# topling/toplingdb

Hardware: NVIDIA H100
Metric: compaction_input_kv_MB_per_s (higher is better)
Workload: dtype u8

## Files before the change

toplingdb_b200/csrc/api.cu:

```cuda
#include <cuda_runtime.h>
#include <stdio.h>
#include <stdlib.h>
#include <string.h>

#include <algorithm>
#include <map>
#include <memory>
#include <mutex>
#include <unordered_map>
#include <string>
#include <thread>
#include <type_traits>
#include <vector>

#include "../../include/b200c.h"
#include "inflate_rules.h"
#include "kernels.h"
#include "range_plan.h"
#include "scan.cuh"
#include "sst_host.h"

using namespace b200c;

namespace {
// ... 190 lines not shown
  cudaEvent_t a, b;
  float us;
};

}

struct b200c_job {
  b200c_params p;
  std::vector<uint64_t> snapshots, fct;
  std::string cf_name, db_id, db_session_id, db_host_id;
  std::vector<Input> inputs;
  std::vector<Output> outputs;
  b200c_stats stats;
  int stage_done = 0;
  uint64_t launches = 0;
  int sms = 132;
  cudaStream_t st = nullptr;
  cudaStream_t st2 = nullptr;
  cudaStream_t st_up = nullptr;
  cudaEvent_t ev[5] = {nullptr, nullptr, nullptr, nullptr, nullptr};
  cudaEvent_t evx[4] = {nullptr, nullptr, nullptr, nullptr};
  DevBuf files_d, blk_off, blk_size, blk_state, scan_tmp, run_start, small;
  KeyBufs dec, mrg;
  DevBuf splits, tile_state, snaps_d;
  DevBuf esz, eshared, tstat, nxt, disk, rows, tstate, grows, gstate, gflag, gsync, idx_contrib, idx_contrib_off, blocks, files_rec, idx_esz, idx_eoff, idx_sep, out_buf, out_base_d;
  uint64_t n_total = 0, n_out = 0, nblk_in = 0, nblocks_out = 0;
  uint32_t nfiles_out = 0, nruns = 0;
  DevBuf bloom_contrib, bloom_contrib_off;
  DevBuf bloom_hashes;
  DevBuf kv_arena, kv_offs, kv_klens;
  DevBuf run_bounds, run_first_d;
  std::vector<uint64_t> run_start_h;
  HostBuf host_out;
  std::vector<GpKey> gp_small, gp_large;
  std::vector<uint64_t> gp_size;
  std::vector<uint8_t> gp_same;
  DevBuf gp_keys_d, gp_ranks_d, gp_size_d, gp_same_d, gp_cuts_d;
  BoundKey range_lo{}, range_hi{};
  DevBuf clip_d;
  DevBuf cslot, cslot_off, arena;
  std::vector<cudaEvent_t> range_events;
  std::vector<std::string> range_bounds;
  cudaEvent_t wait_ev = nullptr;
  DevBuf vfiles_d, vrun_start;
  HostBuf pin_small, pin_tails, pin_rd, pin_up;
  size_t pin_up_used = 0;
  std::vector<KernelTime> ktimes;
// ... 721 lines not shown
  uint32_t maxb = 0;
  for (auto& f : fds) maxb = std::max(maxb, f.nblocks);
  if (nblk) {
    j->kt_begin("decode.index");
    launch_index_decode(files_d, k, maxb, j->blk_off.as<uint64_t>(), j->blk_size.as<uint32_t>(), j->range_lo, P.has_range_start, j->range_hi,
                        P.has_range_end, err, st);
    j->kt_end();
    j->launches++;
  }
  const uint8_t* arena = nullptr;
  if (nblk && any_compressed) {
    CU(j->cslot.reserve(4 * (nblk + 1)));
    CU(j->cslot_off.reserve(8 * (nblk + 1)));
    j->kt_begin("decode.inflate");
    launch_block_usize(files_d, j->blk_off.as<uint64_t>(), j->blk_size.as<uint32_t>(), (uint32_t)nblk, j->cslot.as<uint32_t>(), err, st);
    exclusive_scan<uint32_t>(j->cslot.as<uint32_t>(), j->cslot_off.as<uint64_t>(), nblk, j->scan_tmp.as<uint64_t>(), small + kSlotArena, st, &j->launches);
    uint64_t hc[kSmallSlots];
    if (int rc = checked_sync(j, hc)) return rc;
    CU(j->arena.reserve(hc[kSlotArena] + 256));
    arena = j->arena.as<uint8_t>();
    launch_inflate_blocks(files_d, j->blk_off.as<uint64_t>(), j->blk_size.as<uint32_t>(), j->cslot.as<uint32_t>(), j->cslot_off.as<uint64_t>(),
                          (uint32_t)nblk, j->arena.as<uint8_t>(), P.verify_input_checksums, err, j->sms, st);
    j->kt_end();
    j->launches += 3;
  }
  CU(cudaMemsetAsync(j->run_start.p, 0, 8 * (k + 1), st));
  if (nblk) {
    CU(cudaMemsetAsync(j->blk_state.p, 0, 8 * (nblk + 1), st));
    j->kt_begin("decode.blocks");
    launch_block_decode_fused(files_d, k, j->blk_off.as<uint64_t>(), j->blk_size.as<uint32_t>(), (uint32_t)nblk, P.verify_input_checksums, N,
                              j->dec.mut(), j->blk_state.as<unsigned long long>(), reinterpret_cast<uint32_t*>(small + kSlotDecTicket),
                              j->run_start.as<uint64_t>(), small + kSlotTotalIn, err, j->sms, st, arena);
    j->kt_end();
    j->launches++;
  }
  CU(cudaEventRecord(j->ev[1], st));
  const KeyCols decc = j->dec.cols(N);
  if (until == 1) {
    uint64_t h[kSmallSlots];
    j->run_start_h.resize(k + 1);
    CU(cudaMemcpyAsync(j->run_start_h.data(), j->run_start.p, 8 * (k + 1), cudaMemcpyDeviceToHost, st));
    if (int rc = checked_sync(j, h)) return rc;
    if (h[kSlotTotalIn] != N && !(P.has_range_start || P.has_range_end))
      return fail(B200C_ERR_CORRUPTION, "decoded entry count differs from rocksdb.num.entries");
    j->stage_done = 1;
    j->stats.kernel_launches = j->launches;
    return B200C_OK;
// ... 20 lines not shown
    j->kt_begin("merge.clip");
    launch_clip_runs(decc, runs, K, j->range_lo, P.has_range_start, j->range_hi, P.has_range_end,
                     j->clip_d.as<uint64_t>(), reinterpret_cast<unsigned long long*>(small + kSlotClip), st);
    j->kt_end();
    j->launches++;
    uint64_t hc[kSmallSlots];
    if (int rc = checked_sync(j, hc)) return rc;
    N_in = hc[kSlotClip];
    range_value_bytes = hc[kSlotClip + 1];
    if (N_in > n_decoded) return fail(B200C_ERR_CUDA, "internal: clipped entry count exceeds the input");
    runs = RunBounds{j->clip_d.as<uint64_t>(), j->clip_d.as<uint64_t>() + K};
    j->stats.num_input_records = N_in;
  }
  return run_merge_encode(j, until, decc, runs, n_decoded, N_in, clipped, range_value_bytes, small, err);
}

int run_merge_encode(b200c_job* j, int until, KeyCols decc, RunBounds runs, uint64_t n_decoded, uint64_t N, bool clipped,
                     uint64_t range_value_bytes, uint64_t* small, uint32_t* err) {
  const b200c_params& P = j->p;
  cudaStream_t st = j->st;
  const size_t k = j->nruns;
  const uint64_t mtiles = (N + kMergeNominal - 1) / kMergeNominal;
  CU(j->splits.reserve(8 * (mtiles + 1) * k));
  CU(j->tile_state.reserve(8 * (mtiles + 1)));
  CU(cudaMemsetAsync(j->tile_state.p, 0, 8 * (mtiles + 1), st));
  CU(j->snaps_d.reserve(8 * (P.num_snapshots + 1)));
  if (P.num_snapshots)
    if (int rc = upload_small(j, j->snaps_d.p, j->snapshots.data(), 8 * P.num_snapshots)) return rc;
  CU(j->mrg.reserve(N));
  CU(j->esz.reserve(4 * (N + 1)));
  CU(j->eshared.reserve(N + 1));
  CU(j->tstat.reserve(sizeof(TileStat) * (mtiles + 2)));
  MergeParams mp;
  mp.nruns = (uint32_t)k;
  mp.bottommost = P.bottommost_level != 0;
  mp.nsnapshots = P.num_snapshots;
  mp.snapshots = j->snaps_d.as<uint64_t>();
  mp.earliest_snapshot = P.num_snapshots ? j->snapshots[0] : kMaxSeq;
  mp.filter = P.compaction_filter;
  mp.ttl = P.ttl;
  mp.now = P.ttl_now;
  mp.write_conflict_snapshot = P.earliest_write_conflict_snapshot != 0 && P.earliest_write_conflict_snapshot < kMaxSeq;
  MergeCounters* counters = reinterpret_cast<MergeCounters*>(small + kSlotCounters);
  EncodeWork W;
  memset(&W, 0, sizeof W);
  W.esz = j->esz.as<uint32_t>();
  W.eshared = j->eshared.as<uint8_t>();
  W.tstat = j->tstat.as<TileStat>();
  W.min_s1 = reinterpret_cast<uint32_t*>(small + kSlotMinS1);
  W.totals = small + kSlotTotals;
  if (N) {
    j->kt_begin("merge.partition");
    launch_merge_partition(decc, runs, (uint32_t)k, N, mtiles, j->splits.as<uint64_t>(), err, j->sms, st);
    j->kt_end();
    const MergeSizes msz{W.esz, W.eshared, W.tstat, W.min_s1};
    W.tprefix = j->tile_state.as<unsigned long long>();
    W.nstat = mtiles;
    j->kt_begin("merge.tiles");
    launch_merge_tiles(decc, runs, mp, N, mtiles, j->splits.as<uint64_t>(),
                       j->tile_state.as<unsigned long long>(), reinterpret_cast<uint32_t*>(small + kSlotTicket), j->mrg.mut(), counters, msz, err, st);
    j->kt_end();
    j->kt_begin("merge.sizes_fix");
    launch_merge_sizes_fix(j->mrg.cols(0), j->tile_state.as<unsigned long long>(), mtiles, msz, st);
    j->kt_end();
    j->launches += 3;
  }
  CU(cudaEventRecord(j->ev[2], st));
  uint64_t h[kSmallSlots];
  if (int rc = checked_sync(j, h)) return rc;
  if (clipped ? h[kSlotTotalIn] > n_decoded : h[kSlotTotalIn] != n_decoded)
    return fail(B200C_ERR_CORRUPTION, "decoded entry count differs from rocksdb.num.entries");
  MergeCounters mc;
  memcpy(&mc, h + kSlotCounters, sizeof mc);
  const uint64_t n_out = mc.n_out;
  j->n_out = n_out;
  j->stats.num_output_records = n_out;
  j->stats.num_input_deletion_records = mc.n_input_deletions;
  j->stats.num_records_replaced = mc.n_hidden;
  j->stats.num_expired_deletion_records = mc.n_obsolete;
  j->stats.num_record_drop_user = mc.n_user_drop;
  j->stats.total_input_raw_key_bytes = mc.raw_key_bytes;
  {
    uint64_t all = 0;
    for (auto& in : j->inputs) all += in.tail.raw_value_size;
    if (clipped) all = range_value_bytes;
    j->stats.total_input_raw_value_bytes = all - mc.raw_value_bytes;
  }
  if (until == 2) {
// ... 547 lines not shown
```

toplingdb_b200/csrc/kernels.h:

```cpp
#pragma once
#include <cuda_runtime.h>
#include <stdint.h>

#include <atomic>

#include "common.cuh"
#include "gp_rules.h"

namespace b200c {

struct PerDeviceFlag {
  std::atomic<uint64_t> mask{0};
  uint64_t bit_of_current_device() const {
    int d = 0;
    cudaGetDevice(&d);
    return 1ull << (d & 63);
  }
  bool is_set(uint64_t bit) const { return (mask.load(std::memory_order_acquire) & bit) != 0; }
  void set(uint64_t bit) { mask.fetch_or(bit, std::memory_order_release); }
};

struct FileDesc {
  const uint8_t* base;
  uint64_t len;
// ... 54 lines not shown
  int64_t now;
  uint32_t write_conflict_snapshot;
};
struct TileStat {
  uint64_t raw_key, raw_value, deletions, smallest_seq, largest_seq;
};
struct MergeSizes {
  uint32_t* esz;
  uint8_t* eshared;
  TileStat* tstat;
  uint32_t* min_s1;
};
struct MergeCounters {
  unsigned long long n_out, n_input_deletions, n_hidden, n_obsolete, raw_key_bytes, raw_value_bytes, n_silent, n_user_drop;
};
struct RunBounds {
  const uint64_t* begin;
  const uint64_t* end;
};
void launch_clip_runs(KeyCols in, RunBounds runs, uint32_t nruns, BoundKey start, uint32_t has_start, BoundKey end,
                      uint32_t has_end, uint64_t* clip, unsigned long long* totals, cudaStream_t st);
void launch_run_bounds(KeyCols in, const uint64_t* file_start, const uint32_t* run_first, uint32_t nruns, uint64_t* bounds, uint32_t* err,
                       cudaStream_t st);
void launch_merge_partition(KeyCols in, RunBounds runs, uint32_t nruns, uint64_t n_total, uint64_t ntiles,
                            uint64_t* splits, uint32_t* err, int sms, cudaStream_t st);
void launch_merge_tiles(KeyCols in, RunBounds runs, MergeParams mp, uint64_t n_total, uint64_t ntiles,
                        const uint64_t* splits, unsigned long long* tile_state, uint32_t* ticket, KeyColsMut out,
                        MergeCounters* counters, MergeSizes ms, uint32_t* err, cudaStream_t st);
void launch_merge_sizes_fix(KeyCols merged, const unsigned long long* tile_state, uint64_t ntiles, MergeSizes ms, cudaStream_t st);

struct GpCut {
  uint64_t entry;
  uint64_t block_bytes;
};
struct EncodeParams {
  uint32_t block_size, block_size_limit , restart_interval;
  uint32_t checksum, format_version, output_level;
  uint64_t max_output_file_size;
  GpCtx gp;
  GpCut* gp_cuts;
  uint32_t* gp_ncuts;
};
using GpKey = BoundKey;
void launch_bloom_count(KeyCols m, uint64_t n, FileRec* files, const uint64_t* nfiles_dev, uint32_t millibits, uint64_t* hashes, int sms, cudaStream_t st);
void launch_bloom_build(const uint64_t* hashes, uint64_t n, const FileRec* files, uint32_t nfiles, uint32_t max_filter_bytes, uint32_t millibits, uint32_t cksum,
                        uint8_t* const* out_base, uint64_t* contrib, const uint64_t* contrib_off, cudaStream_t st);
void launch_gp_ranks(KeyCols m, const GpKey* smallest, const GpKey* largest, uint32_t n, uint64_t* lo, uint64_t* eq, uint64_t* hi,
                     cudaStream_t st);
// ... 84 lines not shown
```

toplingdb_b200/csrc/merge.cu:

```cuda
#include "common.cuh"
#include "group_rules.h"
#include "kernels.h"

namespace b200c {

constexpr int kMT = kMergeTile;
constexpr int kMThreads = 256;
constexpr int kMV = kMT / kMThreads;

__device__ __forceinline__ Key load_key(const KeyCols& c, uint64_t i) {
  Key k;
  ulonglong2 p = c.pfx[i];
  k.hi = p.x;
  k.lo = p.y;
  k.tr = c.tr[i];
  k.ulen = meta_ulen(c.meta[i]);
  return k;
}

__device__ __forceinline__ uint64_t count_before(const KeyCols& c, uint64_t base, uint64_t lo, uint64_t hi, const Key& x,
                                                 bool before_equal) {
  while (lo < hi) {
    uint64_t mid = lo + ((hi - lo) >> 1);
    Key e = load_key(c, base + mid);
    bool precedes = before_equal ? !ikey_less(x, e) : ikey_less(e, x);
    if (precedes) lo = mid + 1;
    else hi = mid;
  }
  return lo;
}

__global__ void __launch_bounds__(128)
merge_partition_kernel(KeyCols in, RunBounds runs, uint32_t nruns, uint64_t n_total, uint64_t ntiles,
                       uint64_t* __restrict__ splits, uint32_t* __restrict__ err) {
  const unsigned lane = threadIdx.x & 31;
  const uint64_t b = (uint64_t)blockIdx.x * (blockDim.x >> 5) + (threadIdx.x >> 5);
  if (b > ntiles) return;
  uint64_t d = b * (uint64_t)kMergeNominal;
  if (d > n_total) d = n_total;
  uint64_t base[2], lo[2], hi[2];
#pragma unroll
  for (int s = 0; s < 2; s++) {
    uint32_t r = lane + 32 * s;
    base[s] = r < nruns ? runs.begin[r] : 0;
    uint64_t n = r < nruns ? runs.end[r] - runs.begin[r] : 0;
    lo[s] = (d == n_total) ? n : 0;
    hi[s] = (d == 0) ? 0 : n;
  }
  for (int guard = 0; guard < 64 * 70; guard++) {
    unsigned long long best = 0;
#pragma unroll
    for (int s = 0; s < 2; s++) {
      unsigned long long wdt = hi[s] - lo[s];
      unsigned long long enc = (wdt << 7) | (unsigned long long)(lane + 32 * s);
      if (wdt && enc > best) best = enc;
    }
#pragma unroll
    for (int dd = 16; dd; dd >>= 1) {
      unsigned long long o = __shfl_xor_sync(0xffffffffu, best, dd);
      if (o > best) best = o;
    }
    if (best == 0) break;
    const uint32_t p = (uint32_t)(best & 127);
    const int ps = p >> 5, pl = p & 31;
    uint64_t m = ps ? (lo[1] + ((hi[1] - lo[1]) >> 1)) : (lo[0] + ((hi[0] - lo[0]) >> 1));
    m = __shfl_sync(0xffffffffu, m, pl);
    uint64_t pbase = __shfl_sync(0xffffffffu, ps ? base[1] : base[0], pl);
    const Key x = load_key(in, pbase + m);
    uint64_t c[2], sum = 0;
#pragma unroll
    for (int s = 0; s < 2; s++) {
      uint32_t r = lane + 32 * s;
      if (r == p) c[s] = m;
      else if (r < nruns) c[s] = count_before(in, base[s], lo[s], hi[s], x, r < p);
      else c[s] = 0;
      sum += c[s];
    }
#pragma unroll
    for (int dd = 16; dd; dd >>= 1) sum += __shfl_xor_sync(0xffffffffu, sum, dd);
    const bool x_before = sum < d;
#pragma unroll
    for (int s = 0; s < 2; s++) {
      uint32_t r = lane + 32 * s;
      if (r >= nruns) continue;
      if (x_before) lo[s] = (r == p) ? m + 1 : c[s];
      else hi[s] = (r == p) ? m : c[s];
    }
  }
  uint64_t tot = lo[0] + lo[1];
#pragma unroll
  for (int dd = 16; dd; dd >>= 1) tot += __shfl_xor_sync(0xffffffffu, tot, dd);
  if (tot != d && lane == 0) atomicOr(err, kErrKeyOrder);
  if (lane == 0 && (*reinterpret_cast<volatile uint32_t*>(err) & (uint32_t)kFlagHasSingleDelete)) atomicOr(err, (uint32_t)kErrGroupTooLong);
#pragma unroll
  for (int s = 0; s < 2; s++) {
    uint32_t r = lane + 32 * s;
    if (r < nruns) splits[b * nruns + r] = lo[s];
  }
}

constexpr uint32_t kPartStride = 64;
struct GroupLanes {
  uint32_t gshift, g, r, sub, gbase, nruns;
};
__device__ __forceinline__ bool entry_precedes(const KeyCols& c, uint64_t i, const Key& x, bool before_equal) {
  const ulonglong2 p = c.pfx[i];
  if (p.x != x.hi) return p.x < x.hi;
  if (p.y != x.lo) return p.y < x.lo;
  const uint32_t ul = meta_ulen(c.meta[i]);
  if (ul != x.ulen) return ul < x.ulen;
  const uint64_t tr = c.tr[i];
  if (tr != x.tr) return tr > x.tr;
  return before_equal;
}
__device__ __forceinline__ void msel_grouped(const KeyCols& in, const GroupLanes& L, uint64_t base, uint64_t stride, uint64_t d, uint64_t& lo,
                                             uint64_t& hi) {
  const uint32_t g = L.g, r = L.r, sub = L.sub, gbase = L.gbase, gshift = L.gshift;
  for (int guard = 0; guard < 64 * 70; guard++) {
    const unsigned long long wdt = hi - lo;
    unsigned long long best = wdt ? ((wdt << 7) | (unsigned long long)r) : 0;
#pragma unroll
    for (int dd = 16; dd; dd >>= 1) {
      const unsigned long long o = __shfl_xor_sync(0xffffffffu, best, dd);
      if (o > best) best = o;
    }
    if (best == 0) break;
    const uint32_t p = (uint32_t)(best & 127);
    const uint64_t m = __shfl_sync(0xffffffffu, lo + ((hi - lo) >> 1), (int)(p << gshift));
    const uint64_t pbase = __shfl_sync(0xffffffffu, base, (int)(p << gshift));
    const Key x = load_key(in, pbase + m * stride);
    const bool before_equal = r < p;
    uint64_t clo = lo, chi = hi;
    if (r == p) clo = chi = m;
    while (__any_sync(0xffffffffu, chi > clo)) {
      const uint64_t w = chi - clo;
      uint64_t pos = clo;
      bool valid = false;
      if (w > 0) {
        if (w <= g) {
          pos = clo + sub;
          valid = sub < w;
        } else {
          pos = clo + (w * (sub + 1)) / (g + 1);
          valid = true;
        }
      }
      bool prec = false;
      if (valid) prec = entry_precedes(in, base + pos * stride, x, before_equal);
      const unsigned bal = __ballot_sync(0xffffffffu, prec);
      const uint32_t cp = __popc((bal >> gbase) & ((1u << g) - 1u));
      const uint32_t nvalid = w == 0 ? 0 : (w <= g ? (uint32_t)w : g);
      const uint64_t below = __shfl_sync(0xffffffffu, pos, (int)(gbase + (cp ? cp - 1 : 0)));
      const uint64_t above = __shfl_sync(0xffffffffu, pos, (int)(gbase + (cp < g ? cp : g - 1)));
      if (w > 0) {
        if (cp) clo = below + 1;
        if (cp < nvalid) chi = above;
        else if (w <= g) chi = clo;
      }
    }
    const uint64_t c = clo;
    uint64_t sum = sub == 0 ? c : 0;
#pragma unroll
    for (int dd = 16; dd; dd >>= 1) sum += __shfl_xor_sync(0xffffffffu, sum, dd);
    const bool x_before = sum < d;
    if (r < L.nruns) {
      if (x_before) lo = (r == p) ? m + 1 : c;
      else hi = (r == p) ? m : c;
    }
  }
}
__global__ void __launch_bounds__(128, 12)
merge_partition_grouped_kernel(KeyCols in, RunBounds runs, uint32_t nruns, uint32_t gshift, uint64_t n_total,
                               uint64_t ntiles, uint64_t* __restrict__ splits, uint32_t* __restrict__ err, uint32_t chunk) {
  const unsigned lane = threadIdx.x & 31;
  const uint64_t b0 = ((uint64_t)blockIdx.x * (blockDim.x >> 5) + (threadIdx.x >> 5)) * chunk;
  if (b0 > ntiles) return;
  GroupLanes L;
  L.gshift = gshift;
  L.g = 1u << gshift;
  L.r = lane >> gshift;
  L.sub = lane & (L.g - 1);
  L.gbase = L.r << gshift;
  L.nruns = nruns;
  const uint32_t r = L.r, sub = L.sub;
  const uint64_t base = r < nruns ? runs.begin[r] : 0;
  const uint64_t nrun = r < nruns ? runs.end[r] - runs.begin[r] : 0;
  uint64_t prev_lo = 0, prev_d = 0;
  const bool sd_mode = (*reinterpret_cast<volatile uint32_t*>(err) & (uint32_t)kFlagHasSingleDelete) != 0;
  for (uint32_t c = 0; c < chunk; c++) {
    const uint64_t b = b0 + c;
    if (b > ntiles) break;
    uint64_t d = b * (uint64_t)kMergeNominal;
    if (d > n_total) d = n_total;
    uint64_t lo = (d == n_total) ? nrun : 0, hi = (d == 0) ? 0 : nrun;
    if (d != 0 && d != n_total) {
      if (c != 0) {
        lo = prev_lo;
        hi = d > prev_d ? (prev_lo + (d - prev_d) < nrun ? prev_lo + (d - prev_d) : nrun) : prev_lo;
      } else {
        const uint64_t S = kPartStride, msamp = (nrun + S - 1) / S;
        uint64_t M = sub == 0 ? msamp : 0;
#pragma unroll
        for (int dd = 16; dd; dd >>= 1) M += __shfl_xor_sync(0xffffffffu, M, dd);
        const uint64_t T_lo = d / S, T_hi = (d + (S - 1) * (uint64_t)nruns + S - 1) / S;
        uint64_t tlo = 0, tlo_hi = msamp;
        if (T_lo > 0) msel_grouped(in, L, base, S, T_lo, tlo, tlo_hi);
        if (tlo) lo = S * tlo - (S - 1);
        if (T_hi < M) {
          uint64_t thi = tlo, thi_hi = tlo + (T_hi - T_lo) < msamp ? tlo + (T_hi - T_lo) : msamp;
          msel_grouped(in, L, base, S, T_hi, thi, thi_hi);
          const uint64_t h = S * thi;
          hi = h < nrun ? h : nrun;
        }
        if (hi < lo) hi = lo;
      }
    }
    msel_grouped(in, L, base, 1, d, lo, hi);
    uint64_t tot = sub == 0 ? lo : 0;
#pragma unroll
    for (int dd = 16; dd; dd >>= 1) tot += __shfl_xor_sync(0xffffffffu, tot, dd);
    if (tot != d && lane == 0) atomicOr(err, kErrKeyOrder);
    if (sd_mode && d != 0 && d != n_total) {
      Key head, tail;
      head.hi = head.lo = ~0ull, head.ulen = 0xffffffffu, head.tr = 0;
      tail.hi = tail.lo = 0, tail.ulen = 0, tail.tr = ~0ull;
      const bool have_head = r < nruns && sub == 0 && lo < nrun, have_tail = r < nruns && sub == 0 && lo > 0;
      if (have_head) head = load_key(in, base + lo);
      if (have_tail) tail = load_key(in, base + lo - 1);
      Key mh = head, mt = tail;
      bool anyh = have_head, anyt = have_tail;
#pragma unroll
      for (int dd = 16; dd; dd >>= 1) {
        Key oh, ot;
        oh.hi = __shfl_xor_sync(0xffffffffu, mh.hi, dd), oh.lo = __shfl_xor_sync(0xffffffffu, mh.lo, dd), oh.ulen = __shfl_xor_sync(0xffffffffu, mh.ulen, dd);
        ot.hi = __shfl_xor_sync(0xffffffffu, mt.hi, dd), ot.lo = __shfl_xor_sync(0xffffffffu, mt.lo, dd), ot.ulen = __shfl_xor_sync(0xffffffffu, mt.ulen, dd);
        const bool ohv = __shfl_xor_sync(0xffffffffu, (int)anyh, dd) != 0, otv = __shfl_xor_sync(0xffffffffu, (int)anyt, dd) != 0;
        if (ohv && (!anyh || ukey_cmp(oh.hi, oh.lo, oh.ulen, mh.hi, mh.lo, mh.ulen) < 0)) mh = oh, anyh = true;
        if (otv && (!anyt || ukey_cmp(ot.hi, ot.lo, ot.ulen, mt.hi, mt.lo, mt.ulen) > 0)) mt = ot, anyt = true;
      }
      if (anyh && anyt && ukey_cmp(mh.hi, mh.lo, mh.ulen, mt.hi, mt.lo, mt.ulen) == 0) {
        uint32_t adv = 0;
        if (r < nruns && sub == 0) {
          while (lo < nrun && adv <= (uint32_t)kSdSpill) {
            const ulonglong2 p = in.pfx[base + lo];
            if (!same_ukey(mh, p.x, p.y, meta_ulen(in.meta[base + lo]))) break;
            lo++;
            adv++;
          }
        }
        uint32_t tadv = adv;
#pragma unroll
        for (int dd = 16; dd; dd >>= 1) tadv += __shfl_xor_sync(0xffffffffu, tadv, dd);
        if (tadv > (uint32_t)kSdSpill && lane == 0) atomicOr(err, (uint32_t)kErrGroupTooLong);
        d += tadv;
        lo = __shfl_sync(0xffffffffu, lo, (int)L.gbase);
      }
    }
    if (r < nruns && sub == 0) splits[b * nruns + r] = lo;
    prev_lo = lo;
    prev_d = d;
  }
}

constexpr uint32_t kSnapCache = 16;
struct TileSmem {
  uint64_t hi[kMT], lo[kMT], tr[kMT];
  uint16_t idx[kMT];
  uint8_t ulen[kMT];
  uint8_t verd[kMT];
  uint32_t seg[kMaxRuns + 1];
  uint32_t lst[2][kMaxRuns + 2];
  uint64_t sbeg[kMaxRuns];
  uint64_t snaps[kSnapCache];
  unsigned long long red[8];
  unsigned long long stat[5];
  uint32_t smin, smax;
  uint32_t wsum[40];
  uint64_t base_out;
  uint32_t tile_id, kept_total;
  Key pred;
  uint32_t has_pred;
};

__device__ __forceinline__ Key skey(const TileSmem& s, uint32_t id) {
  Key k;
// ... 707 lines not shown
  if ((threadIdx.x & 31) == 0 && sum) atomicAdd(&totals[1], sum);
}
void launch_clip_runs(KeyCols in, RunBounds runs, uint32_t nruns, BoundKey start, uint32_t has_start, BoundKey end,
                      uint32_t has_end, uint64_t* clip, unsigned long long* totals, cudaStream_t st) {
  if (nruns) clip_runs_kernel<<<dim3(kClipSlices, nruns), 256, 0, st>>>(in, runs, nruns, start, has_start, end, has_end, clip, totals);
}
__global__ void run_bounds_kernel(KeyCols in, const uint64_t* __restrict__ file_start, const uint32_t* __restrict__ run_first, uint32_t nruns,
                                  uint64_t* __restrict__ bounds, uint32_t* __restrict__ err) {
  const uint32_t r = blockIdx.x * blockDim.x + threadIdx.x;
  if (r >= nruns) return;
  const uint32_t f0 = run_first[r], f1 = run_first[r + 1];
  bounds[r] = file_start[f0];
  bounds[nruns + r] = file_start[f1];
  for (uint32_t f = f0 + 1; f < f1; f++) {
    const uint64_t e = file_start[f];
    if (e > file_start[f0] && e < file_start[f1] && !ikey_less(load_key(in, e - 1), load_key(in, e))) atomicOr(err, (uint32_t)kErrKeyOrder);
  }
}
void launch_run_bounds(KeyCols in, const uint64_t* file_start, const uint32_t* run_first, uint32_t nruns, uint64_t* bounds, uint32_t* err,
                       cudaStream_t st) {
  if (nruns) run_bounds_kernel<<<(nruns + 63) / 64, 64, 0, st>>>(in, file_start, run_first, nruns, bounds, err);
}

void launch_merge_partition(KeyCols in, RunBounds runs, uint32_t nruns, uint64_t n_total, uint64_t ntiles,
                            uint64_t* splits, uint32_t* err, int sms, cudaStream_t st) {
  unsigned warps = (unsigned)(ntiles + 1);
  if (nruns <= 16) {
    uint32_t kp2 = 2;
    while (kp2 < nruns) kp2 <<= 1;
    uint32_t gshift = 0;
    while ((kp2 << (gshift + 1)) <= 32) gshift++;
    const unsigned wave = (unsigned)sms * 48u;
    uint32_t chunk = (uint32_t)((warps + wave - 1) / wave);
    if (chunk > 4) chunk = 4;
    if (chunk < 1) chunk = 1;
    const unsigned chunks = (warps + chunk - 1) / chunk;
    merge_partition_grouped_kernel<<<(chunks + 3) / 4, 128, 0, st>>>(in, runs, nruns, gshift, n_total, ntiles, splits, err, chunk);
    return;
  }
  merge_partition_kernel<<<(warps + 3) / 4, 128, 0, st>>>(in, runs, nruns, n_total, ntiles, splits, err);
}
static_assert(sizeof(Key) * kMaxRuns <= sizeof(uint64_t) * kMT && 4 * kMaxRuns <= 2 * kMT, "candidate staging must fit");
static_assert(kMergeCtasPerSm * (sizeof(TileSmem) + 1024) <= 227 * 1024, "merge tile must fit three CTAs per SM");
void launch_merge_tiles(KeyCols in, RunBounds runs, MergeParams mp, uint64_t n_total, uint64_t ntiles,
                        const uint64_t* splits, unsigned long long* tile_state, uint32_t* ticket, KeyColsMut out,
                        MergeCounters* counters, MergeSizes ms, uint32_t* err, cudaStream_t st) {
  if (ntiles == 0) return;
  static PerDeviceFlag attr;
  const uint64_t dev_bit = attr.bit_of_current_device();
  if (!attr.is_set(dev_bit)) {
    cudaFuncSetAttribute(merge_tiles_kernel<false>, cudaFuncAttributeMaxDynamicSharedMemorySize, (int)sizeof(TileSmem));
    cudaFuncSetAttribute(merge_tiles_kernel<true>, cudaFuncAttributeMaxDynamicSharedMemorySize, (int)sizeof(TileSmem));
    attr.set(dev_bit);
  }
  merge_tiles_kernel<false><<<(unsigned)ntiles, kMThreads, sizeof(TileSmem), st>>>(in, runs, mp, n_total, ntiles, splits, tile_state, ticket,
                                                                                   out, counters, ms, err);
  merge_tiles_kernel<true><<<(unsigned)ntiles, kMThreads, sizeof(TileSmem), st>>>(in, runs, mp, n_total, ntiles, splits, tile_state, ticket,
                                                                                  out, counters, ms, err);
}
void launch_merge_sizes_fix(KeyCols merged, const unsigned long long* tile_state, uint64_t ntiles, MergeSizes ms, cudaStream_t st) {
  if (ntiles) merge_sizes_fix_kernel<<<(unsigned)((ntiles + 127) / 128), 128, 0, st>>>(merged, tile_state, ntiles, ms);
}

// ... 2 lines not shown
```

Baseline: 281,800.

## Pre-sort sampled fence keys to bound merge partition searches

Replaces the per-tile multi-way selection over sampled keys with a global fence array. Every 64th key of each run is gathered and merged pairwise across runs over log2(nruns) rounds. Each partition warp then indexes the sorted fences directly to get tight per-run bounds before the exact selection. This removes repeated sample-level selection work per tile, at the cost of extra scratch memory and several extra kernel launches.

```diff
diff --git a/toplingdb_b200/csrc/api.cu b/toplingdb_b200/csrc/api.cu
--- a/toplingdb_b200/csrc/api.cu
+++ b/toplingdb_b200/csrc/api.cu
@@ -236,7 +236,7 @@
   cudaEvent_t evx[4] = {nullptr, nullptr, nullptr, nullptr};
   DevBuf files_d, blk_off, blk_size, blk_state, scan_tmp, run_start, small;
   KeyBufs dec, mrg;
-  DevBuf splits, tile_state, snaps_d;
+  DevBuf splits, fences, tile_state, snaps_d;
   DevBuf esz, eshared, tstat, nxt, disk, rows, tstate, grows, gstate, gflag, gsync, idx_contrib, idx_contrib_off, blocks, files_rec, idx_esz, idx_eoff, idx_sep, out_buf, out_base_d;
   uint64_t n_total = 0, n_out = 0, nblk_in = 0, nblocks_out = 0;
   uint32_t nfiles_out = 0, nruns = 0;
@@ -1004,7 +1004,7 @@
     launch_inflate_blocks(files_d, j->blk_off.as<uint64_t>(), j->blk_size.as<uint32_t>(), j->cslot.as<uint32_t>(), j->cslot_off.as<uint64_t>(),
                           (uint32_t)nblk, j->arena.as<uint8_t>(), P.verify_input_checksums, err, j->sms, st);
     j->kt_end();
-    j->launches += 3;
+    j->launches += 2;
   }
   CU(cudaMemsetAsync(j->run_start.p, 0, 8 * (k + 1), st));
   if (nblk) {
@@ -1071,6 +1071,7 @@
   const size_t k = j->nruns;
   const uint64_t mtiles = (N + kMergeNominal - 1) / kMergeNominal;
   CU(j->splits.reserve(8 * (mtiles + 1) * k));
+  CU(j->fences.reserve(merge_partition_scratch_bytes((uint32_t)k, N)));
   CU(j->tile_state.reserve(8 * (mtiles + 1)));
   CU(cudaMemsetAsync(j->tile_state.p, 0, 8 * (mtiles + 1), st));
   CU(j->snaps_d.reserve(8 * (P.num_snapshots + 1)));
@@ -1100,7 +1101,7 @@
   W.totals = small + kSlotTotals;
   if (N) {
     j->kt_begin("merge.partition");
-    launch_merge_partition(decc, runs, (uint32_t)k, N, mtiles, j->splits.as<uint64_t>(), err, j->sms, st);
+    j->launches += launch_merge_partition(decc, runs, (uint32_t)k, N, mtiles, j->fences.p, j->splits.as<uint64_t>(), err, st);
     j->kt_end();
     const MergeSizes msz{W.esz, W.eshared, W.tstat, W.min_s1};
     W.tprefix = j->tile_state.as<unsigned long long>();
@@ -1112,7 +1113,7 @@
     j->kt_begin("merge.sizes_fix");
     launch_merge_sizes_fix(j->mrg.cols(0), j->tile_state.as<unsigned long long>(), mtiles, msz, st);
     j->kt_end();
-    j->launches += 3;
+    j->launches += 2;
   }
   CU(cudaEventRecord(j->ev[2], st));
   uint64_t h[kSmallSlots];
diff --git a/toplingdb_b200/csrc/kernels.h b/toplingdb_b200/csrc/kernels.h
--- a/toplingdb_b200/csrc/kernels.h
+++ b/toplingdb_b200/csrc/kernels.h
@@ -100,8 +100,9 @@
                       uint32_t has_end, uint64_t* clip, unsigned long long* totals, cudaStream_t st);
 void launch_run_bounds(KeyCols in, const uint64_t* file_start, const uint32_t* run_first, uint32_t nruns, uint64_t* bounds, uint32_t* err,
                        cudaStream_t st);
-void launch_merge_partition(KeyCols in, RunBounds runs, uint32_t nruns, uint64_t n_total, uint64_t ntiles,
-                            uint64_t* splits, uint32_t* err, int sms, cudaStream_t st);
+size_t merge_partition_scratch_bytes(uint32_t nruns, uint64_t n_total);
+int launch_merge_partition(KeyCols in, RunBounds runs, uint32_t nruns, uint64_t n_total, uint64_t ntiles, void* scratch,
+                           uint64_t* splits, uint32_t* err, cudaStream_t st);
 void launch_merge_tiles(KeyCols in, RunBounds runs, MergeParams mp, uint64_t n_total, uint64_t ntiles,
                         const uint64_t* splits, unsigned long long* tile_state, uint32_t* ticket, KeyColsMut out,
                         MergeCounters* counters, MergeSizes ms, uint32_t* err, cudaStream_t st);
diff --git a/toplingdb_b200/csrc/merge.cu b/toplingdb_b200/csrc/merge.cu
--- a/toplingdb_b200/csrc/merge.cu
+++ b/toplingdb_b200/csrc/merge.cu
@@ -30,151 +30,242 @@
   return lo;
 }
 
-__global__ void __launch_bounds__(128)
-merge_partition_kernel(KeyCols in, RunBounds runs, uint32_t nruns, uint64_t n_total, uint64_t ntiles,
-                       uint64_t* __restrict__ splits, uint32_t* __restrict__ err) {
+constexpr uint32_t kPartStride = 64;
+constexpr int kFenceWin = 1024;
+constexpr int kFenceThreads = 256;
+
+struct FenceCols {
+  ulonglong2* pfx;
+  uint64_t* tr;
+  uint32_t* ulen;
+  uint32_t* ord[2];
+  uint64_t* foff;
+};
+__device__ __forceinline__ Key fence_key(const FenceCols& fc, uint64_t f) {
+  Key k;
+  const ulonglong2 p = fc.pfx[f];
+  k.hi = p.x;
+  k.lo = p.y;
+  k.tr = fc.tr[f];
+  k.ulen = fc.ulen[f];
+  return k;
+}
+__device__ __forceinline__ uint32_t fence_at(const uint32_t* ord, uint64_t i) { return ord ? ord[i] : (uint32_t)i; }
+
+__global__ void __launch_bounds__(kFenceThreads)
+merge_fence_gather_kernel(KeyCols in, RunBounds runs, uint32_t nruns, FenceCols fc) {
+  __shared__ uint64_t foff[kMaxRuns + 1];
+  if (threadIdx.x < nruns) foff[threadIdx.x + 1] = (runs.end[threadIdx.x] - runs.begin[threadIdx.x] + kPartStride - 1) / kPartStride;
+  __syncthreads();
+  if (threadIdx.x == 0) {
+    foff[0] = 0;
+    for (uint32_t r = 0; r < nruns; r++) foff[r + 1] += foff[r];
+  }
+  __syncthreads();
+  if (blockIdx.x == 0 && threadIdx.x <= nruns) fc.foff[threadIdx.x] = foff[threadIdx.x];
+  const uint64_t f = (uint64_t)blockIdx.x * blockDim.x + threadIdx.x;
+  if (f >= foff[nruns]) return;
+  uint32_t r = 0;
+  for (uint32_t step = kMaxRuns; step; step >>= 1)
+    if (r + step <= nruns && foff[r + step] <= f) r += step;
+  const Key k = load_key(in, runs.begin[r] + kPartStride * (f - foff[r]));
+  fc.pfx[f] = make_ulonglong2(k.hi, k.lo);
+  fc.tr[f] = k.tr;
+  fc.ulen[f] = k.ulen;
+}
+
+__global__ void __launch_bounds__(kFenceThreads)
+merge_fence_round_kernel(FenceCols fc, uint32_t nruns, uint32_t t) {
+  __shared__ uint64_t foff[kMaxRuns + 1];
+  __shared__ uint32_t win[kMaxRuns / 2 + 1];
+  __shared__ uint64_t split[2];
+  __shared__ uint64_t s_hi[kFenceWin], s_lo[kFenceWin], s_tr[kFenceWin];
+  __shared__ uint32_t s_ulen[kFenceWin], s_f[kFenceWin];
+  const uint32_t* src = t == 0 ? nullptr : (t & 1) ? fc.ord[0] : fc.ord[1];
+  uint32_t* dst = (t & 1) ? fc.ord[1] : fc.ord[0];
+  const uint32_t w = 1u << t, npairs = (nruns + 2 * w - 1) / (2 * w);
+  if (threadIdx.x <= nruns) foff[threadIdx.x] = fc.foff[threadIdx.x];
+  __syncthreads();
+  if (threadIdx.x == 0) {
+    win[0] = 0;
+    for (uint32_t i = 0; i < npairs; i++) {
+      const uint32_t r1 = min((i + 1) * 2 * w, nruns);
+      win[i + 1] = win[i] + (uint32_t)((foff[r1] - foff[i * 2 * w] + kFenceWin - 1) / kFenceWin);
+    }
+  }
+  __syncthreads();
+  if (blockIdx.x >= win[npairs]) return;
+  uint32_t i = 0;
+  while (win[i + 1] <= blockIdx.x) i++;
+  const uint32_t rm = min((2 * i + 1) * w, nruns), r1 = min((2 * i + 2) * w, nruns);
+  const uint64_t A0 = foff[2 * i * w], A = foff[rm] - A0, B0 = foff[rm], B = foff[r1] - B0;
+  const uint64_t o0 = (uint64_t)(blockIdx.x - win[i]) * kFenceWin, o1 = min(o0 + kFenceWin, A + B);
+  if (threadIdx.x < 2) {
+    const uint64_t o = threadIdx.x ? o1 : o0;
+    uint64_t lo = o > B ? o - B : 0, hi = min(o, A);
+    while (lo < hi) {
+      const uint64_t mid = lo + ((hi - lo) >> 1);
+      if (!ikey_less(fence_key(fc, fence_at(src, B0 + o - mid - 1)), fence_key(fc, fence_at(src, A0 + mid)))) lo = mid + 1;
+      else hi = mid;
+    }
+    split[threadIdx.x] = lo;
+  }
+  __syncthreads();
+  const uint64_t a0 = split[0], b0 = o0 - a0;
+  const uint32_t na = (uint32_t)(split[1] - a0), n = (uint32_t)(o1 - o0);
+  for (uint32_t x = threadIdx.x; x < n; x += blockDim.x) {
+    const uint32_t f = fence_at(src, x < na ? A0 + a0 + x : B0 + b0 + (x - na));
+    const Key k = fence_key(fc, f);
+    s_hi[x] = k.hi, s_lo[x] = k.lo, s_tr[x] = k.tr, s_ulen[x] = k.ulen, s_f[x] = f;
+  }
+  __syncthreads();
+  for (uint32_t x = threadIdx.x; x < n; x += blockDim.x) {
+    const Key k{s_hi[x], s_lo[x], s_tr[x], s_ulen[x]};
+    const bool left = x < na;
+    uint32_t lo = left ? na : 0, hi = left ? n : na;
+    const uint32_t first = lo;
+    while (lo < hi) {
+      const uint32_t mid = (lo + hi) >> 1;
+      const Key e{s_hi[mid], s_lo[mid], s_tr[mid], s_ulen[mid]};
+      if (left ? ikey_less(e, k) : !ikey_less(k, e)) lo = mid + 1;
+      else hi = mid;
+    }
+    dst[A0 + o0 + (left ? x : x - na) + (lo - first)] = s_f[x];
+  }
+}
+
+struct GroupLanes {
+  uint32_t gshift, g, r, sub, gbase, nruns;
+};
+struct RunEntries {
+  const KeyCols& in;
+  uint64_t base;
+  __device__ __forceinline__ bool precedes(uint64_t pos, const Key& x, bool before_equal) const {
+    const uint64_t i = base + pos;
+    const ulonglong2 p = in.pfx[i];
+    if (p.x != x.hi) return p.x < x.hi;
+    if (p.y != x.lo) return p.y < x.lo;
+    const uint32_t ul = meta_ulen(in.meta[i]);
+    if (ul != x.ulen) return ul < x.ulen;
+    const uint64_t tr = in.tr[i];
+    if (tr != x.tr) return tr > x.tr;
+    return before_equal;
+  }
+};
+struct RunFences {
+  const FenceCols& fc;
+  uint64_t base;
+  __device__ __forceinline__ bool precedes(uint64_t pos, const Key& x, bool before_equal) const {
+    const uint64_t f = base + pos;
+    const ulonglong2 p = fc.pfx[f];
+    if (p.x != x.hi) return p.x < x.hi;
+    if (p.y != x.lo) return p.y < x.lo;
+    const uint32_t ul = fc.ulen[f];
+    if (ul != x.ulen) return ul < x.ulen;
+    const uint64_t tr = fc.tr[f];
+    if (tr != x.tr) return tr > x.tr;
+    return before_equal;
+  }
+};
+template <class Src>
+__device__ __forceinline__ uint64_t group_count(const Src& src, const GroupLanes& L, uint32_t r, uint64_t lo, uint64_t hi, const Key& x,
+                                                uint32_t p, uint64_t m) {
+  const uint32_t g = L.g, sub = L.sub, gbase = L.gbase;
+  const bool before_equal = r < p;
+  uint64_t clo = lo, chi = hi;
+  if (r == p) clo = chi = m;
+  while (__any_sync(0xffffffffu, chi > clo)) {
+    const uint64_t w = chi - clo;
+    uint64_t pos = clo;
+    bool valid = false;
+    if (w > 0) {
+      if (w <= g) {
+        pos = clo + sub;
+        valid = sub < w;
+      } else {
+        pos = clo + (w * (sub + 1)) / (g + 1);
+        valid = true;
+      }
+    }
+    bool prec = false;
+    if (valid) prec = src.precedes(pos, x, before_equal);
+    const unsigned bal = __ballot_sync(0xffffffffu, prec);
+    const uint32_t cp = __popc((bal >> gbase) & ((1u << g) - 1u));
+    const uint32_t nvalid = w == 0 ? 0 : (w <= g ? (uint32_t)w : g);
+    const uint64_t below = __shfl_sync(0xffffffffu, pos, (int)(gbase + (cp ? cp - 1 : 0)));
+    const uint64_t above = __shfl_sync(0xffffffffu, pos, (int)(gbase + (cp < g ? cp : g - 1)));
+    if (w > 0) {
+      if (cp) clo = below + 1;
+      if (cp < nvalid) chi = above;
+      else if (w <= g) chi = clo;
+    }
+  }
+  return clo;
+}
+template <int RPL>
+__device__ __forceinline__ void msel_grouped(const KeyCols& in, const GroupLanes& L, const uint64_t (&base)[RPL], uint64_t d,
+                                             uint64_t (&lo)[RPL], uint64_t (&hi)[RPL]) {
+  for (int guard = 0; guard < 64 * 70; guard++) {
+    unsigned long long best = 0;
+#pragma unroll
+    for (int s = 0; s < RPL; s++) {
+      const unsigned long long wdt = hi[s] - lo[s];
+      const unsigned long long e = wdt ? ((wdt << 7) | (unsigned long long)(L.r + 32 * s)) : 0;
+      if (e > best) best = e;
+    }
+#pragma unroll
+    for (int dd = 16; dd; dd >>= 1) {
+      const unsigned long long o = __shfl_xor_sync(0xffffffffu, best, dd);
+      if (o > best) best = o;
+    }
+    if (best == 0) break;
+    const uint32_t p = (uint32_t)(best & 127);
+    const bool ps = RPL > 1 && p >= 32;
+    const int pl = RPL > 1 ? (int)(p & 31) : (int)(p << L.gshift);
+    const uint64_t m = __shfl_sync(0xffffffffu, ps ? lo[RPL - 1] + ((hi[RPL - 1] - lo[RPL - 1]) >> 1) : lo[0] + ((hi[0] - lo[0]) >> 1), pl);
+    const uint64_t pbase = __shfl_sync(0xffffffffu, ps ? base[RPL - 1] : base[0], pl);
+    const Key x = load_key(in, pbase + m);
+    uint64_t c[RPL], sum = 0;
+#pragma unroll
+    for (int s = 0; s < RPL; s++) {
+      c[s] = group_count(RunEntries{in, base[s]}, L, L.r + 32 * s, lo[s], hi[s], x, p, m);
+      if (L.sub == 0) sum += c[s];
+    }
+#pragma unroll
+    for (int dd = 16; dd; dd >>= 1) sum += __shfl_xor_sync(0xffffffffu, sum, dd);
+    const bool x_before = sum < d;
+#pragma unroll
+    for (int s = 0; s < RPL; s++) {
+      const uint32_t r = L.r + 32 * s;
+      if (r >= L.nruns) continue;
+      if (x_before) lo[s] = (r == p) ? m + 1 : c[s];
+      else hi[s] = (r == p) ? m : c[s];
+    }
+  }
+}
+template <int RPL>
+__device__ __forceinline__ void fence_split(const FenceCols& fc, const uint32_t* ord, const GroupLanes& L, const uint64_t (&fb)[RPL],
+                                            const uint64_t (&fe)[RPL], uint64_t T, const uint64_t (&lo)[RPL], const uint64_t (&hi)[RPL],
+                                            uint64_t (&t)[RPL]) {
+  const uint32_t f = fence_at(ord, T);
+  const Key y = fence_key(fc, f);
+  uint32_t p = 0;
+#pragma unroll
+  for (int s = 0; s < RPL; s++) {
+    const unsigned own = __ballot_sync(0xffffffffu, L.sub == 0 && fb[s] <= f && f < fe[s]);
+    if (own) p = ((uint32_t)(__ffs(own) - 1) >> L.gshift) + 32 * s;
+  }
+#pragma unroll
+  for (int s = 0; s < RPL; s++) t[s] = group_count(RunFences{fc, fb[s]}, L, L.r + 32 * s, lo[s], hi[s], y, p, f - fb[s]);
+}
+
+template <int RPL>
+__global__ void __launch_bounds__(128, RPL == 1 ? 12 : 8)
+merge_partition_kernel(KeyCols in, RunBounds runs, uint32_t nruns, uint32_t gshift, uint64_t n_total, uint64_t ntiles, FenceCols fc,
+                       const uint32_t* __restrict__ ord, uint64_t* __restrict__ splits, uint32_t* __restrict__ err) {
   const unsigned lane = threadIdx.x & 31;
   const uint64_t b = (uint64_t)blockIdx.x * (blockDim.x >> 5) + (threadIdx.x >> 5);
   if (b > ntiles) return;
-  uint64_t d = b * (uint64_t)kMergeNominal;
-  if (d > n_total) d = n_total;
-  uint64_t base[2], lo[2], hi[2];
-#pragma unroll
-  for (int s = 0; s < 2; s++) {
-    uint32_t r = lane + 32 * s;
-    base[s] = r < nruns ? runs.begin[r] : 0;
-    uint64_t n = r < nruns ? runs.end[r] - runs.begin[r] : 0;
-    lo[s] = (d == n_total) ? n : 0;
-    hi[s] = (d == 0) ? 0 : n;
-  }
-  for (int guard = 0; guard < 64 * 70; guard++) {
-    unsigned long long best = 0;
-#pragma unroll
-    for (int s = 0; s < 2; s++) {
-      unsigned long long wdt = hi[s] - lo[s];
-      unsigned long long enc = (wdt << 7) | (unsigned long long)(lane + 32 * s);
-      if (wdt && enc > best) best = enc;
-    }
-#pragma unroll
-    for (int dd = 16; dd; dd >>= 1) {
-      unsigned long long o = __shfl_xor_sync(0xffffffffu, best, dd);
-      if (o > best) best = o;
-    }
-    if (best == 0) break;
-    const uint32_t p = (uint32_t)(best & 127);
-    const int ps = p >> 5, pl = p & 31;
-    uint64_t m = ps ? (lo[1] + ((hi[1] - lo[1]) >> 1)) : (lo[0] + ((hi[0] - lo[0]) >> 1));
-    m = __shfl_sync(0xffffffffu, m, pl);
-    uint64_t pbase = __shfl_sync(0xffffffffu, ps ? base[1] : base[0], pl);
-    const Key x = load_key(in, pbase + m);
-    uint64_t c[2], sum = 0;
-#pragma unroll
-    for (int s = 0; s < 2; s++) {
-      uint32_t r = lane + 32 * s;
-      if (r == p) c[s] = m;
-      else if (r < nruns) c[s] = count_before(in, base[s], lo[s], hi[s], x, r < p);
-      else c[s] = 0;
-      sum += c[s];
-    }
-#pragma unroll
-    for (int dd = 16; dd; dd >>= 1) sum += __shfl_xor_sync(0xffffffffu, sum, dd);
-    const bool x_before = sum < d;
-#pragma unroll
-    for (int s = 0; s < 2; s++) {
-      uint32_t r = lane + 32 * s;
-      if (r >= nruns) continue;
-      if (x_before) lo[s] = (r == p) ? m + 1 : c[s];
-      else hi[s] = (r == p) ? m : c[s];
-    }
-  }
-  uint64_t tot = lo[0] + lo[1];
-#pragma unroll
-  for (int dd = 16; dd; dd >>= 1) tot += __shfl_xor_sync(0xffffffffu, tot, dd);
-  if (tot != d && lane == 0) atomicOr(err, kErrKeyOrder);
-  if (lane == 0 && (*reinterpret_cast<volatile uint32_t*>(err) & (uint32_t)kFlagHasSingleDelete)) atomicOr(err, (uint32_t)kErrGroupTooLong);
-#pragma unroll
-  for (int s = 0; s < 2; s++) {
-    uint32_t r = lane + 32 * s;
-    if (r < nruns) splits[b * nruns + r] = lo[s];
-  }
-}
-
-constexpr uint32_t kPartStride = 64;
-struct GroupLanes {
-  uint32_t gshift, g, r, sub, gbase, nruns;
-};
-__device__ __forceinline__ bool entry_precedes(const KeyCols& c, uint64_t i, const Key& x, bool before_equal) {
-  const ulonglong2 p = c.pfx[i];
-  if (p.x != x.hi) return p.x < x.hi;
-  if (p.y != x.lo) return p.y < x.lo;
-  const uint32_t ul = meta_ulen(c.meta[i]);
-  if (ul != x.ulen) return ul < x.ulen;
-  const uint64_t tr = c.tr[i];
-  if (tr != x.tr) return tr > x.tr;
-  return before_equal;
-}
-__device__ __forceinline__ void msel_grouped(const KeyCols& in, const GroupLanes& L, uint64_t base, uint64_t stride, uint64_t d, uint64_t& lo,
-                                             uint64_t& hi) {
-  const uint32_t g = L.g, r = L.r, sub = L.sub, gbase = L.gbase, gshift = L.gshift;
-  for (int guard = 0; guard < 64 * 70; guard++) {
-    const unsigned long long wdt = hi - lo;
-    unsigned long long best = wdt ? ((wdt << 7) | (unsigned long long)r) : 0;
-#pragma unroll
-    for (int dd = 16; dd; dd >>= 1) {
-      const unsigned long long o = __shfl_xor_sync(0xffffffffu, best, dd);
-      if (o > best) best = o;
-    }
-    if (best == 0) break;
-    const uint32_t p = (uint32_t)(best & 127);
-    const uint64_t m = __shfl_sync(0xffffffffu, lo + ((hi - lo) >> 1), (int)(p << gshift));
-    const uint64_t pbase = __shfl_sync(0xffffffffu, base, (int)(p << gshift));
-    const Key x = load_key(in, pbase + m * stride);
-    const bool before_equal = r < p;
-    uint64_t clo = lo, chi = hi;
-    if (r == p) clo = chi = m;
-    while (__any_sync(0xffffffffu, chi > clo)) {
-      const uint64_t w = chi - clo;
-      uint64_t pos = clo;
-      bool valid = false;
-      if (w > 0) {
-        if (w <= g) {
-          pos = clo + sub;
-          valid = sub < w;
-        } else {
-          pos = clo + (w * (sub + 1)) / (g + 1);
-          valid = true;
-        }
-      }
-      bool prec = false;
-      if (valid) prec = entry_precedes(in, base + pos * stride, x, before_equal);
-      const unsigned bal = __ballot_sync(0xffffffffu, prec);
-      const uint32_t cp = __popc((bal >> gbase) & ((1u << g) - 1u));
-      const uint32_t nvalid = w == 0 ? 0 : (w <= g ? (uint32_t)w : g);
-      const uint64_t below = __shfl_sync(0xffffffffu, pos, (int)(gbase + (cp ? cp - 1 : 0)));
-      const uint64_t above = __shfl_sync(0xffffffffu, pos, (int)(gbase + (cp < g ? cp : g - 1)));
-      if (w > 0) {
-        if (cp) clo = below + 1;
-        if (cp < nvalid) chi = above;
-        else if (w <= g) chi = clo;
-      }
-    }
-    const uint64_t c = clo;
-    uint64_t sum = sub == 0 ? c : 0;
-#pragma unroll
-    for (int dd = 16; dd; dd >>= 1) sum += __shfl_xor_sync(0xffffffffu, sum, dd);
-    const bool x_before = sum < d;
-    if (r < L.nruns) {
-      if (x_before) lo = (r == p) ? m + 1 : c;
-      else hi = (r == p) ? m : c;
-    }
-  }
-}
-__global__ void __launch_bounds__(128, 12)
-merge_partition_grouped_kernel(KeyCols in, RunBounds runs, uint32_t nruns, uint32_t gshift, uint64_t n_total,
-                               uint64_t ntiles, uint64_t* __restrict__ splits, uint32_t* __restrict__ err, uint32_t chunk) {
-  const unsigned lane = threadIdx.x & 31;
-  const uint64_t b0 = ((uint64_t)blockIdx.x * (blockDim.x >> 5) + (threadIdx.x >> 5)) * chunk;
-  if (b0 > ntiles) return;
   GroupLanes L;
   L.gshift = gshift;
   L.g = 1u << gshift;
@@ -183,84 +274,97 @@
   L.gbase = L.r << gshift;
   L.nruns = nruns;
   const uint32_t r = L.r, sub = L.sub;
-  const uint64_t base = r < nruns ? runs.begin[r] : 0;
-  const uint64_t nrun = r < nruns ? runs.end[r] - runs.begin[r] : 0;
-  uint64_t prev_lo = 0, prev_d = 0;
+  uint64_t base[RPL], nrun[RPL], lo[RPL], hi[RPL];
+  uint64_t d = b * (uint64_t)kMergeNominal;
+  if (d > n_total) d = n_total;
+#pragma unroll
+  for (int s = 0; s < RPL; s++) {
+    const uint32_t rs = r + 32 * s;
+    base[s] = rs < nruns ? runs.begin[rs] : 0;
+    nrun[s] = rs < nruns ? runs.end[rs] - base[s] : 0;
+    lo[s] = (d == n_total) ? nrun[s] : 0;
+    hi[s] = (d == 0) ? 0 : nrun[s];
+  }
+  if (d != 0 && d != n_total) {
+    const uint64_t S = kPartStride, M = fc.foff[nruns];
+    uint64_t fb[RPL], fe[RPL], nf[RPL], zero[RPL], tlo[RPL], thi[RPL], cap[RPL];
+#pragma unroll
+    for (int s = 0; s < RPL; s++) {
+      const uint32_t rs = r + 32 * s;
+      fb[s] = rs < nruns ? fc.foff[rs] : 0;
+      fe[s] = rs < nruns ? fc.foff[rs + 1] : 0;
+      nf[s] = fe[s] - fb[s];
+      zero[s] = tlo[s] = 0;
+    }
+    const uint64_t T_lo = d / S, T_hi = (d + (S - 1) * (uint64_t)nruns + S - 1) / S;
+    if (T_lo > 0 && T_lo < M) fence_split(fc, ord, L, fb, fe, T_lo, zero, nf, tlo);
+#pragma unroll
+    for (int s = 0; s < RPL; s++) {
+      if (tlo[s]) lo[s] = S * tlo[s] - (S - 1);
+      cap[s] = tlo[s] + (T_hi - T_lo) < nf[s] ? tlo[s] + (T_hi - T_lo) : nf[s];
+    }
+    if (T_hi < M) {
+      fence_split(fc, ord, L, fb, fe, T_hi, tlo, cap, thi);
+#pragma unroll
+      for (int s = 0; s < RPL; s++) {
+        const uint64_t h = S * thi[s];
+        hi[s] = h < nrun[s] ? h : nrun[s];
+      }
+    }
+#pragma unroll
+    for (int s = 0; s < RPL; s++)
+      if (hi[s] < lo[s]) hi[s] = lo[s];
+  }
+  msel_grouped<RPL>(in, L, base, d, lo, hi);
+  uint64_t tot = 0;
+#pragma unroll
+  for (int s = 0; s < RPL; s++)
+    if (sub == 0) tot += lo[s];
+#pragma unroll
+  for (int dd = 16; dd; dd >>= 1) tot += __shfl_xor_sync(0xffffffffu, tot, dd);
+  if (tot != d && lane == 0) atomicOr(err, kErrKeyOrder);
   const bool sd_mode = (*reinterpret_cast<volatile uint32_t*>(err) & (uint32_t)kFlagHasSingleDelete) != 0;
-  for (uint32_t c = 0; c < chunk; c++) {
-    const uint64_t b = b0 + c;
-    if (b > ntiles) break;
-    uint64_t d = b * (uint64_t)kMergeNominal;
-    if (d > n_total) d = n_total;
-    uint64_t lo = (d == n_total) ? nrun : 0, hi = (d == 0) ? 0 : nrun;
-    if (d != 0 && d != n_total) {
-      if (c != 0) {
-        lo = prev_lo;
-        hi = d > prev_d ? (prev_lo + (d - prev_d) < nrun ? prev_lo + (d - prev_d) : nrun) : prev_lo;
-      } else {
-        const uint64_t S = kPartStride, msamp = (nrun + S - 1) / S;
-        uint64_t M = sub == 0 ? msamp : 0;
-#pragma unroll
-        for (int dd = 16; dd; dd >>= 1) M += __shfl_xor_sync(0xffffffffu, M, dd);
-        const uint64_t T_lo = d / S, T_hi = (d + (S - 1) * (uint64_t)nruns + S - 1) / S;
-        uint64_t tlo = 0, tlo_hi = msamp;
-        if (T_lo > 0) msel_grouped(in, L, base, S, T_lo, tlo, tlo_hi);
-        if (tlo) lo = S * tlo - (S - 1);
-        if (T_hi < M) {
-          uint64_t thi = tlo, thi_hi = tlo + (T_hi - T_lo) < msamp ? tlo + (T_hi - T_lo) : msamp;
-          msel_grouped(in, L, base, S, T_hi, thi, thi_hi);
-          const uint64_t h = S * thi;
-          hi = h < nrun ? h : nrun;
+  if (sd_mode && nruns > 16) {
+    if (lane == 0) atomicOr(err, (uint32_t)kErrGroupTooLong);
+  } else if (sd_mode && d != 0 && d != n_total) {
+    Key head, tail;
+    head.hi = head.lo = ~0ull, head.ulen = 0xffffffffu, head.tr = 0;
+    tail.hi = tail.lo = 0, tail.ulen = 0, tail.tr = ~0ull;
+    const bool have_head = r < nruns && sub == 0 && lo[0] < nrun[0], have_tail = r < nruns && sub == 0 && lo[0] > 0;
+    if (have_head) head = load_key(in, base[0] + lo[0]);
+    if (have_tail) tail = load_key(in, base[0] + lo[0] - 1);
+    Key mh = head, mt = tail;
+    bool anyh = have_head, anyt = have_tail;
+#pragma unroll
+    for (int dd = 16; dd; dd >>= 1) {
+      Key oh, ot;
+      oh.hi = __shfl_xor_sync(0xffffffffu, mh.hi, dd), oh.lo = __shfl_xor_sync(0xffffffffu, mh.lo, dd), oh.ulen = __shfl_xor_sync(0xffffffffu, mh.ulen, dd);
+      ot.hi = __shfl_xor_sync(0xffffffffu, mt.hi, dd), ot.lo = __shfl_xor_sync(0xffffffffu, mt.lo, dd), ot.ulen = __shfl_xor_sync(0xffffffffu, mt.ulen, dd);
+      const bool ohv = __shfl_xor_sync(0xffffffffu, (int)anyh, dd) != 0, otv = __shfl_xor_sync(0xffffffffu, (int)anyt, dd) != 0;
+      if (ohv && (!anyh || ukey_cmp(oh.hi, oh.lo, oh.ulen, mh.hi, mh.lo, mh.ulen) < 0)) mh = oh, anyh = true;
+      if (otv && (!anyt || ukey_cmp(ot.hi, ot.lo, ot.ulen, mt.hi, mt.lo, mt.ulen) > 0)) mt = ot, anyt = true;
+    }
+    if (anyh && anyt && ukey_cmp(mh.hi, mh.lo, mh.ulen, mt.hi, mt.lo, mt.ulen) == 0) {
+      uint32_t adv = 0;
+      if (r < nruns && sub == 0) {
+        while (lo[0] < nrun[0] && adv <= (uint32_t)kSdSpill) {
+          const ulonglong2 p = in.pfx[base[0] + lo[0]];
+          if (!same_ukey(mh, p.x, p.y, meta_ulen(in.meta[base[0] + lo[0]]))) break;
+          lo[0]++;
+          adv++;
         }
-        if (hi < lo) hi = lo;
       }
-    }
-    msel_grouped(in, L, base, 1, d, lo, hi);
-    uint64_t tot = sub == 0 ? lo : 0;
-#pragma unroll
-    for (int dd = 16; dd; dd >>= 1) tot += __shfl_xor_sync(0xffffffffu, tot, dd);
-    if (tot != d && lane == 0) atomicOr(err, kErrKeyOrder);
-    if (sd_mode && d != 0 && d != n_total) {
-      Key head, tail;
-      head.hi = head.lo = ~0ull, head.ulen = 0xffffffffu, head.tr = 0;
-      tail.hi = tail.lo = 0, tail.ulen = 0, tail.tr = ~0ull;
-      const bool have_head = r < nruns && sub == 0 && lo < nrun, have_tail = r < nruns && sub == 0 && lo > 0;
-      if (have_head) head = load_key(in, base + lo);
-      if (have_tail) tail = load_key(in, base + lo - 1);
-      Key mh = head, mt = tail;
-      bool anyh = have_head, anyt = have_tail;
-#pragma unroll
-      for (int dd = 16; dd; dd >>= 1) {
-        Key oh, ot;
-        oh.hi = __shfl_xor_sync(0xffffffffu, mh.hi, dd), oh.lo = __shfl_xor_sync(0xffffffffu, mh.lo, dd), oh.ulen = __shfl_xor_sync(0xffffffffu, mh.ulen, dd);
-        ot.hi = __shfl_xor_sync(0xffffffffu, mt.hi, dd), ot.lo = __shfl_xor_sync(0xffffffffu, mt.lo, dd), ot.ulen = __shfl_xor_sync(0xffffffffu, mt.ulen, dd);
-        const bool ohv = __shfl_xor_sync(0xffffffffu, (int)anyh, dd) != 0, otv = __shfl_xor_sync(0xffffffffu, (int)anyt, dd) != 0;
-        if (ohv && (!anyh || ukey_cmp(oh.hi, oh.lo, oh.ulen, mh.hi, mh.lo, mh.ulen) < 0)) mh = oh, anyh = true;
-        if (otv && (!anyt || ukey_cmp(ot.hi, ot.lo, ot.ulen, mt.hi, mt.lo, mt.ulen) > 0)) mt = ot, anyt = true;
-      }
-      if (anyh && anyt && ukey_cmp(mh.hi, mh.lo, mh.ulen, mt.hi, mt.lo, mt.ulen) == 0) {
-        uint32_t adv = 0;
-        if (r < nruns && sub == 0) {
-          while (lo < nrun && adv <= (uint32_t)kSdSpill) {
-            const ulonglong2 p = in.pfx[base + lo];
-            if (!same_ukey(mh, p.x, p.y, meta_ulen(in.meta[base + lo]))) break;
-            lo++;
-            adv++;
-          }
-        }
-        uint32_t tadv = adv;
-#pragma unroll
-        for (int dd = 16; dd; dd >>= 1) tadv += __shfl_xor_sync(0xffffffffu, tadv, dd);
-        if (tadv > (uint32_t)kSdSpill && lane == 0) atomicOr(err, (uint32_t)kErrGroupTooLong);
-        d += tadv;
-        lo = __shfl_sync(0xffffffffu, lo, (int)L.gbase);
-      }
-    }
-    if (r < nruns && sub == 0) splits[b * nruns + r] = lo;
-    prev_lo = lo;
-    prev_d = d;
-  }
-}
+      uint32_t tadv = adv;
+#pragma unroll
+      for (int dd = 16; dd; dd >>= 1) tadv += __shfl_xor_sync(0xffffffffu, tadv, dd);
+      if (tadv > (uint32_t)kSdSpill && lane == 0) atomicOr(err, (uint32_t)kErrGroupTooLong);
+    }
+  }
+#pragma unroll
+  for (int s = 0; s < RPL; s++)
+    if (r + 32 * s < nruns && sub == 0) splits[b * nruns + r + 32 * s] = lo[s];
+}
+
 
 constexpr uint32_t kSnapCache = 16;
 struct TileSmem {
@@ -1014,23 +1118,42 @@
   if (nruns) run_bounds_kernel<<<(nruns + 63) / 64, 64, 0, st>>>(in, file_start, run_first, nruns, bounds, err);
 }
 
-void launch_merge_partition(KeyCols in, RunBounds runs, uint32_t nruns, uint64_t n_total, uint64_t ntiles,
-                            uint64_t* splits, uint32_t* err, int sms, cudaStream_t st) {
-  unsigned warps = (unsigned)(ntiles + 1);
-  if (nruns <= 16) {
+static uint64_t fence_cap(uint32_t nruns, uint64_t n_total) { return n_total / kPartStride + nruns; }
+size_t merge_partition_scratch_bytes(uint32_t nruns, uint64_t n_total) {
+  return (sizeof(ulonglong2) + sizeof(uint64_t) + 3 * sizeof(uint32_t)) * fence_cap(nruns, n_total) + sizeof(uint64_t) * (kMaxRuns + 1);
+}
+int launch_merge_partition(KeyCols in, RunBounds runs, uint32_t nruns, uint64_t n_total, uint64_t ntiles, void* scratch,
+                           uint64_t* splits, uint32_t* err, cudaStream_t st) {
+  const uint64_t cap = fence_cap(nruns, n_total);
+  FenceCols fc;
+  fc.pfx = static_cast<ulonglong2*>(scratch);
+  fc.tr = reinterpret_cast<uint64_t*>(fc.pfx + cap);
+  fc.foff = fc.tr + cap;
+  fc.ulen = reinterpret_cast<uint32_t*>(fc.foff + kMaxRuns + 1);
+  fc.ord[0] = fc.ulen + cap;
+  fc.ord[1] = fc.ord[0] + cap;
+  int launches = 0;
+  merge_fence_gather_kernel<<<(unsigned)((cap + kFenceThreads - 1) / kFenceThreads), kFenceThreads, 0, st>>>(in, runs, nruns, fc);
+  launches++;
+  uint32_t rounds = 0;
+  while ((1u << rounds) < nruns) rounds++;
+  for (uint32_t t = 0; t < rounds; t++) {
+    const unsigned grid = (unsigned)((cap + kFenceWin - 1) / kFenceWin) + (nruns + (2u << t) - 1) / (2u << t);
+    merge_fence_round_kernel<<<grid, kFenceThreads, 0, st>>>(fc, nruns, t);
+    launches++;
+  }
+  const uint32_t* ord = rounds ? fc.ord[(rounds - 1) & 1] : nullptr;
+  const unsigned ctas = (unsigned)((ntiles + 1 + 3) / 4);
+  if (nruns <= 32) {
     uint32_t kp2 = 2;
     while (kp2 < nruns) kp2 <<= 1;
     uint32_t gshift = 0;
     while ((kp2 << (gshift + 1)) <= 32) gshift++;
-    const unsigned wave = (unsigned)sms * 48u;
-    uint32_t chunk = (uint32_t)((warps + wave - 1) / wave);
-    if (chunk > 4) chunk = 4;
-    if (chunk < 1) chunk = 1;
-    const unsigned chunks = (warps + chunk - 1) / chunk;
-    merge_partition_grouped_kernel<<<(chunks + 3) / 4, 128, 0, st>>>(in, runs, nruns, gshift, n_total, ntiles, splits, err, chunk);
-    return;
-  }
-  merge_partition_kernel<<<(warps + 3) / 4, 128, 0, st>>>(in, runs, nruns, n_total, ntiles, splits, err);
+    merge_partition_kernel<1><<<ctas, 128, 0, st>>>(in, runs, nruns, gshift, n_total, ntiles, fc, ord, splits, err);
+  } else {
+    merge_partition_kernel<2><<<ctas, 128, 0, st>>>(in, runs, nruns, 0, n_total, ntiles, fc, ord, splits, err);
+  }
+  return launches + 1;
 }
 static_assert(sizeof(Key) * kMaxRuns <= sizeof(uint64_t) * kMT && 4 * kMaxRuns <= 2 * kMT, "candidate staging must fit");
 static_assert(kMergeCtasPerSm * (sizeof(TileSmem) + 1024) <= 227 * 1024, "merge tile must fit three CTAs per SM");
```

Result: no change. 284,100, median of 6 (+0.8%).
